# vadimkantorov/convasr

Measured on AMD Instinct MI355X. Metric: audio-seconds/sec/node (fwd+bwd+CTC) at bs64x15s, higher is better.
Workload: dtype bf16

## Files before the change

### convasr_amd/csrc/conv.hip

```cpp
#include "conv_common.h"

template <typename T, bool ALIGNED> __device__ __forceinline__ uint4 load_chunk(const T* row, int e0, int n_valid) {
	constexpr int EPC = 16 / sizeof(T);
	uint4 v = make_uint4(0, 0, 0, 0);
	if (ALIGNED) {
		if (e0 + EPC <= n_valid) v = *reinterpret_cast<const uint4*>(row + e0);
		else if (e0 < n_valid) {
			T tmp[EPC];
#pragma unroll
			for (int i = 0; i < EPC; ++i) tmp[i] = (e0 + i < n_valid) ? row[e0 + i] : (T)0;
			v = *reinterpret_cast<uint4*>(tmp);
		}
	} else if (e0 < n_valid) {
		T tmp[EPC];
#pragma unroll
		for (int i = 0; i < EPC; ++i) tmp[i] = (e0 + i < n_valid) ? row[e0 + i] : (T)0;
		v = *reinterpret_cast<uint4*>(tmp);
	}
	return v;
}

template <typename T, typename O, int XI, bool ALIGNED_X, bool SK = false>
__global__ __launch_bounds__(NTHREADS, sizeof(T) == 4 ? 1 : 2) void conv1d_igemm_kernel(ConvParams p) {
	extern __shared__ __attribute__((aligned(16))) char smem[];
// ... 337 lines not shown
	else return convasr_fail(CONVASR_EUNSUPPORTED, "pack_conv_weight: dtype %d", dtype);
	if (rc) return rc;
	CONVASR_CHECK_LAUNCH("pack_conv_weight");
	return 0;
}

template <typename T, typename O, int XI, bool AL, bool SK = false> static int launch_conv(const ConvParams& p, size_t smem, hipStream_t s) {
	auto kern = conv1d_igemm_kernel<T, O, XI, AL, SK>;
	static unsigned long long attr_set = 0;
	convasr_allow_160k_lds(reinterpret_cast<const void*>(kern), attr_set);
	constexpr int BK = ROW_BYTES / sizeof(T);
	const int splits = SK ? ((p.Cin + BK - 1) / BK + p.cib_per_split - 1) / p.cib_per_split : 1;
	hipLaunchKernelGGL(kern, dim3(p.total_tiles, splits), dim3(NTHREADS), smem, s, p);
	return 0;
}

template <typename T, typename O, bool SK = false> static int dispatch_conv(const ConvParams& p, size_t smem, hipStream_t s) {
	const int xi = (p.x_rows * 8 + NTHREADS - 1) / NTHREADS;
	const bool al = ((p.Cin * sizeof(T)) & 15) == 0;
	if (!al) {
		if (xi <= 9) return launch_conv<T, O, 9, false, SK>(p, smem, s);
		return convasr_fail(CONVASR_EUNSUPPORTED, "conv1d: halo too large (x_rows %d)", p.x_rows);
	}
	if (xi <= 5) return launch_conv<T, O, 5, true, SK>(p, smem, s);
	if (xi <= 9) return launch_conv<T, O, 9, true, SK>(p, smem, s);
	if (xi <= 16) return launch_conv<T, O, 16, true, SK>(p, smem, s);
	return convasr_fail(CONVASR_EUNSUPPORTED, "conv1d: halo too large (x_rows %d)", p.x_rows);
}

int convasr_conv1d_v2_try(ConvParams p, int x_dtype, int y_dtype, hipStream_t s, int* m_tiles_out);
int convasr_conv1x1_try(ConvParams p, int x_dtype, int y_dtype, hipStream_t s, int* rows_out);
int convasr_wgrad_v2_try(WgradParams& p, int dtype, hipStream_t s);
int convasr_wgrad_v2_supports(const WgradParams& p);
static int g_conv_use_v2 = 1;
static int g_conv_debug = 0;
int convasr_conv_debug_bits() { return g_conv_debug; }
extern "C" int convasr_debug_set_conv_v2(int enable) { const int prev = g_conv_use_v2; g_conv_use_v2 = enable & 1; g_conv_debug = enable >> 8; return prev; }

static int conv1d_run(const void* x, const void* wp, void* y, int x_dtype, int y_dtype, int B, int Cin, int Cout, int Tin, int Tout, int K,
                      int stride, int dil, int pad, const float* bias, double* stats, const float* scale, const float* shift, int act,
                      float act_lo, float act_hi, const float* xlen, const ConvParams* bn_fusion, int* rows_out, void* stream) {
	CONVASR_CHECK_ARG(x && wp && y && B > 0 && Cin > 0 && Cout > 0 && Tin > 0 && Tout > 0 && K > 0 && stride > 0 && dil > 0, "conv1d_fwd: bad arguments");
	CONVASR_CHECK_ARG((scale == nullptr) == (shift == nullptr), "conv1d_fwd: scale and shift go together");
	const int64_t expect = ((int64_t)Tin + 2 * (int64_t)pad - (int64_t)dil * (K - 1) - 1) / stride + 1;
	CONVASR_CHECK_ARG(Tout <= expect, "conv1d_fwd: Tout %d inconsistent with Tin %d K %d stride %d dil %d pad %d (at most %lld)", Tout, Tin, K, stride, dil, pad, (long long)expect);
	CONVASR_CHECK_ARG(x_dtype == CONVASR_F32 || convasr_is_half(x_dtype), "conv1d_fwd: x dtype %d", x_dtype);
	if (K == 1 && stride == 1 && pad == 0 && Tin == Tout && B > 1 && !xlen && !(bn_fusion && bn_fusion->bn_xlen) && !(g_conv_debug & 512) &&
	    (int64_t)B * Tin * (Cin > Cout ? Cin : Cout) * 4 < (1ll << 31)) {
		Tin = Tout = B * Tin;
		B = 1;
	}
	ConvParams p = {};
	if (bn_fusion) p = *bn_fusion;
	p.x = x; p.w = wp; p.y = y; p.bias = bias; p.stats = stats; p.scale = scale; p.shift = shift; p.xlen = xlen;
	p.B = B; p.Cin = Cin; p.Cout = Cout; p.CoutPad = convasr_conv_cout_pad(Cout); p.Tin = Tin; p.Tout = Tout; p.K = K; p.stride = stride; p.dil = dil; p.pad = pad;
	p.act = act; p.act_lo = act_lo; p.act_hi = act_hi; p.debug = g_conv_debug;
	p.m_tiles_per_b = (Tout + BM - 1) / BM;
	p.n_tiles = p.CoutPad / BN;
	p.total_tiles = B * p.m_tiles_per_b * p.n_tiles;
	int xr = (BM - 1) * stride + (K - 1) * dil + 1;
	p.x_rows = (xr + 1) & ~1;
	const size_t osz = y_dtype == CONVASR_F32 ? 4 : 2;
	size_t smem = 2 * (size_t)p.x_rows * ROW_BYTES + 2 * BN * ROW_BYTES;
	const size_t epi = (size_t)BM * (BN * osz + 16) + 4 * BN * sizeof(float);
	if (epi > smem) smem = epi;
	CONVASR_CHECK_ARG(smem <= 160 * 1024, "conv1d_fwd: tile needs %zu B of LDS", smem);
// ... 350 lines not shown
	double s = 0;
	for (int i = 0; i < 16; ++i) s += red[i][cl];
	out[c] = accumulate ? out[c] + (float)s : (float)s;
}

extern "C" int64_t convasr_colsum_workspace_bytes(int64_t rows, int C) { return ceil_div64(rows, 256) * (int64_t)C * 4; }
extern "C" int convasr_colsum(const void* y, int dtype, int64_t rows, int C, float* out, void* workspace, int accumulate, void* stream) {
	CONVASR_CHECK_ARG(y && out && workspace && rows > 0 && C > 0 && (dtype == CONVASR_F32 || convasr_is_half(dtype)), "colsum: bad arguments");
	hipStream_t s = (hipStream_t)stream;
	const int rows_per_block = 256;
	dim3 grid((C + 63) / 64, (unsigned)ceil_div64(rows, rows_per_block));
	float* part = (float*)workspace;
	if (dtype == CONVASR_F32) hipLaunchKernelGGL((colsum_kernel<float>), grid, dim3(256), 0, s, (const float*)y, part, rows, C, rows_per_block);
	else if (dtype == CONVASR_F16) hipLaunchKernelGGL((colsum_kernel<f16_t>), grid, dim3(256), 0, s, (const f16_t*)y, part, rows, C, rows_per_block);
	else hipLaunchKernelGGL((colsum_kernel<bf16_t>), grid, dim3(256), 0, s, (const bf16_t*)y, part, rows, C, rows_per_block);
	hipLaunchKernelGGL(colsum_final_kernel, dim3((C + 63) / 64), dim3(1024), 0, s, (const float*)part, (int)grid.y, C, out, accumulate);
	CONVASR_CHECK_LAUNCH("colsum");
	return 0;
}

extern "C" int64_t convasr_conv1d_wgrad_workspace_bytes(int B, int Cin, int Cout, int Tin, int Tout, int K, int stride, int dil) {
	WgradParams p;
	p.debug = 0;
	p.B = B; p.Cin = Cin; p.Cout = Cout; p.Tin = Tin; p.Tout = Tout; p.K = K; p.stride = stride; p.dil = dil;
	p.pad = 0;
	int splits = 1;
	const int bkt[3] = {64, WgTile<bf16_t>::BKT, WgTile<float>::BKT};
	const double us[3] = {1.6, 2.7, 11.0};
	for (int i = 0; i < 3; ++i) {
		WgradParams q = p;
		wgrad_plan(q, bkt[i], us[i]);
		if (q.splits > splits) splits = q.splits;
	}
	const int64_t slabs = (int64_t)splits * K * (int64_t)Cout * Cin * 4;
	const int64_t dbias_parts = ceil_div64((int64_t)B * Tout, 256) * Cout * 4;
	return slabs > dbias_parts ? slabs : dbias_parts;
}

template <typename T, int XI, bool AX, bool AY> static void launch_wgrad(const WgradParams& p, size_t smem, hipStream_t s) {
	auto kern = conv1d_wgrad_kernel<T, XI, AX, AY>;
	static unsigned long long attr_set = 0;
	convasr_allow_160k_lds(reinterpret_cast<const void*>(kern), attr_set);
	hipLaunchKernelGGL(kern, dim3(p.units * p.splits), dim3(NTHREADS), smem, s, p);
}

template <typename T> static int dispatch_wgrad(WgradParams& p, hipStream_t s) {
	wgrad_plan(p, WgTile<T>::BKT, sizeof(T) == 2 ? 2.7 : 11.0);
	const int xi = (p.x_rows * WgTile<T>::CPR + NTHREADS - 1) / NTHREADS;
	const size_t smem = 2 * (size_t)(WgTile<T>::BKT + p.x_rows) * WgTile<T>::PITCH;
	if (smem > 160 * 1024 || xi > 12) return convasr_fail(CONVASR_EUNSUPPORTED, "conv1d_wgrad: tile too large (x_rows %d)", p.x_rows);
	const bool ax = ((p.Cin * sizeof(T)) & 15) == 0, ay = ((p.Cout * sizeof(T)) & 15) == 0;
	if (ax && ay) { if (xi <= 5) launch_wgrad<T, 5, true, true>(p, smem, s); else launch_wgrad<T, 12, true, true>(p, smem, s); }
	else if (ax) launch_wgrad<T, 12, true, false>(p, smem, s);
	else if (ay) launch_wgrad<T, 12, false, true>(p, smem, s);
	else launch_wgrad<T, 12, false, false>(p, smem, s);
	return 0;
}

static int wgrad_impl(const void* x, int x_ld, const void* dy, int dy_ld, float* dw, float* dbias, void* workspace, int dtype, int B, int Cin, int Cout, int Tin,
                      int Tout, int K, int stride, int dil, int pad, int accumulate, int dw_layout, void* stream) {
	CONVASR_CHECK_ARG(x && dy && dw && workspace && B > 0 && Cin > 0 && Cout > 0 && Tin > 0 && Tout > 0 && K > 0 && stride > 0 && dil > 0 && (dw_layout == CONVASR_W_REFERENCE || dw_layout == CONVASR_W_KMAJOR), "conv1d_wgrad: bad arguments");
	CONVASR_CHECK_ARG(dw_layout == CONVASR_W_REFERENCE || (((int64_t)Cout * Cin) & 3) == 0, "conv1d_wgrad: K-major dw needs Cout * Cin %% 4 == 0");
	CONVASR_CHECK_ARG(K <= 64, "conv1d_wgrad: K %d > 64", K);
	WgradParams p;
	p.debug = g_conv_debug;
	p.x = x; p.dy = dy; p.slab = (float*)workspace;
// ... 116 lines not shown
```

### convasr_amd/csrc/conv_common.h

```cpp
#pragma once
#include "common.h"

typedef float f32x16 __attribute__((ext_vector_type(16)));
typedef float f32x4 __attribute__((ext_vector_type(4)));
typedef __bf16 bf16x8 __attribute__((ext_vector_type(8)));
typedef _Float16 f16x8 __attribute__((ext_vector_type(8)));

#define BM 128
#define BN 128
#define NTHREADS 256
#define ROW_BYTES 128

struct ConvParams {
	const void* x;
	const void* w;
	void* y;
	const float* bias;
	double* stats;
	const float* scale;
	const float* shift;
	const float* xlen;
	int B, Cin, Cout, CoutPad, Tin, Tout, K, stride, dil, pad;
	int act;
	float act_lo, act_hi;
// ... 56 lines not shown
};
template <> struct Mma<float> {
	static constexpr int EPC = 4;
	__device__ static __forceinline__ void run(const uint4& a, const uint4& b, f32x16& c) {
		c = __builtin_amdgcn_mfma_f32_32x32x2f32(__uint_as_float(a.x), __uint_as_float(b.x), c, 0, 0, 0);
		c = __builtin_amdgcn_mfma_f32_32x32x2f32(__uint_as_float(a.y), __uint_as_float(b.y), c, 0, 0, 0);
		c = __builtin_amdgcn_mfma_f32_32x32x2f32(__uint_as_float(a.z), __uint_as_float(b.z), c, 0, 0, 0);
		c = __builtin_amdgcn_mfma_f32_32x32x2f32(__uint_as_float(a.w), __uint_as_float(b.w), c, 0, 0, 0);
	}
};


template <typename T> struct Mma16;
template <> struct Mma16<bf16_t> {
	template <typename V> __device__ static __forceinline__ f32x4 run(const V& a, const V& b, const f32x4& c) { return __builtin_amdgcn_mfma_f32_16x16x32_bf16(__builtin_bit_cast(bf16x8, a), __builtin_bit_cast(bf16x8, b), c, 0, 0, 0); }
};
template <> struct Mma16<f16_t> {
	template <typename V> __device__ static __forceinline__ f32x4 run(const V& a, const V& b, const f32x4& c) { return __builtin_amdgcn_mfma_f32_16x16x32_f16(__builtin_bit_cast(f16x8, a), __builtin_bit_cast(f16x8, b), c, 0, 0, 0); }
};


#define WG_TG 4

struct WgradParams {
	const void* x;
	const void* dy;
	float* slab;
	int B, Cin, Cout, Tin, Tout, K, stride, dil, pad;
	int co_tiles, ci_tiles, tap_groups, units, splits;
	int chunks_per_b, total_chunks, chunks_per_split;
	int x_rows;
	int debug;
	int x_ld, dy_ld;
};

typedef short s16x4 __attribute__((ext_vector_type(4)));

#define WGRAD_MAX_SPLITS 32

static inline void wgrad_plan(WgradParams& p, int bkt, double chunk_us) {
	p.co_tiles = (p.Cout + 127) / 128;
	p.ci_tiles = (p.Cin + 127) / 128;
	p.tap_groups = (p.K + WG_TG - 1) / WG_TG;
	p.units = p.co_tiles * p.ci_tiles * p.tap_groups;
	p.chunks_per_b = (p.Tout + bkt - 1) / bkt;
	p.total_chunks = p.B * p.chunks_per_b;
	const double slab_us = 2.0 * p.K * (double)p.Cout * p.Cin * 4.0 / 4e6;
	double best = 1e30;
	int best_s = 1;
	for (int s = 1; s <= WGRAD_MAX_SPLITS && s <= p.total_chunks; ++s) {
		const int cps = (p.total_chunks + s - 1) / s, s_eff = (p.total_chunks + cps - 1) / cps;
		const int rounds = (p.units * s_eff + 255) / 256;
		const double cost = rounds * cps * chunk_us + s_eff * slab_us;
		if (cost < best) { best = cost; best_s = s_eff; }
	}
	p.splits = best_s;
	p.chunks_per_split = (p.total_chunks + best_s - 1) / best_s;
	p.splits = (p.total_chunks + p.chunks_per_split - 1) / p.chunks_per_split;
	const int taps = p.K < WG_TG ? p.K : WG_TG;
	p.x_rows = (bkt - 1) * p.stride + (taps - 1) * p.dil + 1;
}
```

### convasr_amd/csrc/wgrad_v2.hip

```cpp
#include "conv_common.h"
#include <type_traits>

#define W2_THREADS 512
#define W2_ALL_THREADS (512 + 256)
#define W2_BKT 64
#define W2_YBYTES (W2_BKT * 256)

typedef int v4i32 __attribute__((ext_vector_type(4)));

#ifdef CONVASR_STAMPS
__device__ unsigned long long g_w2_stamps[256 * 8 * 8];
extern "C" int convasr_debug_read_wgrad_stamps(unsigned long long* host, int count) {
	return hipMemcpyFromSymbol(host, HIP_SYMBOL(g_w2_stamps), sizeof(unsigned long long) * count) == hipSuccess ? 0 : -1;
}
#define WSTAMP(var) { __builtin_amdgcn_sched_barrier(0); asm volatile("s_memtime %0\n\ts_waitcnt lgkmcnt(0)" : "=s"(var) :: "memory"); __builtin_amdgcn_sched_barrier(0); }
#else
#define WSTAMP(var)
#endif

__device__ __forceinline__ v4i32 w2_make_srd(const char* base, unsigned num_bytes) {
	const unsigned long long a = (unsigned long long)base;
	v4i32 d;
	d[0] = __builtin_amdgcn_readfirstlane((int)(unsigned)a);
	d[1] = __builtin_amdgcn_readfirstlane((int)(unsigned)((a >> 32) & 0xffffu));
	d[2] = __builtin_amdgcn_readfirstlane((int)num_bytes);
	d[3] = 0x00020000;
	return d;
}

__device__ __forceinline__ void w2_dma16(const v4i32& srd, unsigned lds_addr, int voff) {
	unsigned keep;
	asm volatile("s_nop 4\n\ts_mov_b32 %0, m0\n\ts_mov_b32 m0, %3\n\ts_nop 0\n\tbuffer_load_dwordx4 %1, %2, 0 offen lds\n\ts_mov_b32 m0, %0"
	             : "=&s"(keep)
	             : "v"(voff), "s"(srd), "s"(lds_addr)
	             : "memory");
}

__device__ __forceinline__ uint4 w2_tr_frag(const char* p0, const char* p1) {
	typedef __attribute__((address_space(3))) s16x4* lp;
	const s16x4 lo = __builtin_amdgcn_ds_read_tr16_b64_v4i16((lp)p0);
	const s16x4 hi = __builtin_amdgcn_ds_read_tr16_b64_v4i16((lp)p1);
	const uint2 l = __builtin_bit_cast(uint2, lo), h = __builtin_bit_cast(uint2, hi);
	return make_uint4(l.x, l.y, h.x, h.y);
}

#define W2_MAX_GROUP 12
struct WgradGroup {
	WgradParams prob[W2_MAX_GROUP];
	int first[W2_MAX_GROUP + 1];
	int n;
};

template <typename H> __device__ __forceinline__ void wgrad_v2_body(const WgradParams& p, const int v, char* const smem) {
	const int tid = threadIdx.x, lane = tid & 63;
	const int wave = __builtin_amdgcn_readfirstlane(tid >> 6);
	const int tp = wave >> 2, wm = (wave >> 1) & 1, wn = wave & 1;

	const int unit = v % p.units, split = v / p.units;
#ifdef CONVASR_AB_WGRAD_ORDER
	int tg, ci_t, co_t;
	{
		const int order = (p.debug >> 13) & 3;
		if (order == 1) { co_t = unit % p.co_tiles; ci_t = (unit / p.co_tiles) % p.ci_tiles; tg = unit / (p.co_tiles * p.ci_tiles); }
		else if (order == 2) {
			const int BS = 3, cb = (p.co_tiles + BS - 1) / BS, ib = (p.ci_tiles + BS - 1) / BS;
			int u = unit, found = 0; tg = ci_t = co_t = 0;
			for (int b0 = 0; b0 < cb * ib && !found; ++b0) {
				const int c0 = (b0 / ib) * BS, i0 = (b0 % ib) * BS;
				const int nc = min(BS, p.co_tiles - c0), ni = min(BS, p.ci_tiles - i0), n = nc * ni * p.tap_groups;
				if (u < n) { tg = u % p.tap_groups; const int r = u / p.tap_groups; ci_t = i0 + r % ni; co_t = c0 + r / ni; found = 1; }
				else u -= n;
			}
		}
		else { tg = unit % p.tap_groups; ci_t = (unit / p.tap_groups) % p.ci_tiles; co_t = unit / (p.tap_groups * p.ci_tiles); }
	}
#else
	const int tg = unit % p.tap_groups, ci_t = (unit / p.tap_groups) % p.ci_tiles, co_t = unit / (p.tap_groups * p.ci_tiles);
#endif
	const int co0 = co_t * 128, ci0 = ci_t * 128, tap0 = tg * WG_TG;
	const int c_begin = split * p.chunks_per_split, c_end = min(p.total_chunks, c_begin + p.chunks_per_split);
	const int ntaps = min(WG_TG, p.K - tap0);
	int tapA, tapB;
	unsigned mA, mB;
	bool shA = false, shB = false;
	if (ntaps == 4) { tapA = tap0 + 2 * tp; tapB = tapA + 1; mA = 15u; mB = 15u; }
	else if (ntaps == 3) { tapA = tap0 + tp; tapB = tap0 + 2; mA = 15u; mB = tp ? 12u : 3u; shB = true; }
	else if (ntaps == 2) { tapA = tap0 + tp; tapB = tapA; mA = 15u; mB = 0u; }
	else { tapA = tap0; tapB = tap0; mA = tp ? 12u : 3u; mB = 0u; shA = true; }

	const int xbytes = p.x_rows * 256;
	const int stage_bytes = W2_YBYTES + xbytes;
	const unsigned lds_base = (unsigned)(size_t)(__attribute__((address_space(3))) char*)smem;
	const int y_row_bytes = (p.dy_ld ? p.dy_ld : p.Cout) * 2, x_row_bytes = (p.x_ld ? p.x_ld : p.Cin) * 2;
	const int y_pieces = W2_BKT / 4, x_pieces = p.x_rows >> 2, pieces = y_pieces + x_pieces;
	const bool loader = wave >= 8;
	const int lw = wave - 8;
	const int my_pieces = (pieces - lw + 3) >> 2;
	const int prow = lane >> 4, pchunk = (lane & 15) ^ (prow << 2);
	const int ylane = prow * y_row_bytes + pchunk * 16 + co0 * 2, xlane = prow * x_row_bytes + pchunk * 16 + ci0 * 2;

	auto issue = [&](int c, int stage) {
		const int b = c / p.chunks_per_b, t0 = (c % p.chunks_per_b) * W2_BKT;
		const v4i32 ysrd = w2_make_srd(reinterpret_cast<const char*>(p.dy) + (int64_t)b * p.Tout * y_row_bytes, (unsigned)(p.Tout * y_row_bytes));
		const v4i32 xsrd = w2_make_srd(reinterpret_cast<const char*>(p.x) + (int64_t)b * p.Tin * x_row_bytes, (unsigned)(p.Tin * x_row_bytes));
		const unsigned dst = lds_base + stage * stage_bytes;
		const int tin0 = t0 - p.pad + tap0 * p.dil;
		for (int j = lw; j < pieces; j += 4) {
			if (j < y_pieces) w2_dma16(ysrd, __builtin_amdgcn_readfirstlane(dst + j * 1024), (t0 + j * 4) * y_row_bytes + ylane);
			else w2_dma16(xsrd, __builtin_amdgcn_readfirstlane(dst + W2_YBYTES + (j - y_pieces) * 1024), (tin0 + (j - y_pieces) * 4) * x_row_bytes + xlane);
		}
	};

	f32x16 acc[2][2][2];
#pragma unroll
	for (int a = 0; a < 2; ++a)
#pragma unroll
		for (int i = 0; i < 2; ++i)
#pragma unroll
			for (int j = 0; j < 2; ++j)
#pragma unroll
				for (int k = 0; k < 16; ++k) acc[a][i][j][k] = 0.f;

	if (loader) {
		for (int i = 0; i < 3; ++i)
			if (c_begin + i < c_end) issue(c_begin + i, i);
		asm volatile("s_waitcnt vmcnt(0)" ::: "memory");
		__builtin_amdgcn_s_barrier();
		int stage = 0;
		for (int c = c_begin; c < c_end; ++c) {
			const bool more = c + 3 < c_end;
			if (more) issue(c + 3, (stage + 3) & 3);
			if (!more) asm volatile("s_waitcnt vmcnt(0)" ::: "memory");
			else switch (my_pieces) {
				case 10: asm volatile("s_waitcnt vmcnt(10)" ::: "memory"); break;
				case 9: asm volatile("s_waitcnt vmcnt(9)" ::: "memory"); break;
				case 8: asm volatile("s_waitcnt vmcnt(8)" ::: "memory"); break;
				case 7: asm volatile("s_waitcnt vmcnt(7)" ::: "memory"); break;
				case 6: asm volatile("s_waitcnt vmcnt(6)" ::: "memory"); break;
				case 5: asm volatile("s_waitcnt vmcnt(5)" ::: "memory"); break;
				default: asm volatile("s_waitcnt vmcnt(0)" ::: "memory"); break;
			}
			__builtin_amdgcn_s_barrier();
			stage = (stage + 1) & 3;
		}
		if (ntaps == 3 || ntaps == 1) __builtin_amdgcn_s_barrier();
		return;
	}
	__builtin_amdgcn_s_barrier();
#ifdef CONVASR_STAMPS
	unsigned long long wa = 0, wb = 0, wc = 0, w_work = 0, w_bar = 0, w_t0 = 0, w_t1 = 0, w_t2 = 0;
	WSTAMP(w_t0)
#endif

	const int g4 = lane >> 4, q = (lane >> 2) & 3, pc = lane & 3;
	const int krow = 8 * (g4 >> 1) + q;
	const int colA = (wm * 64 + (g4 & 1) * 16 + 4 * pc) * 2, colB = (wn * 64 + (g4 & 1) * 16 + 4 * pc) * 2;
	const int offA = (tapA - tap0) * p.dil, offB = (tapB - tap0) * p.dil;
	auto swz = [](int cb, int r3) { return (((cb >> 6) ^ r3) << 6) | (cb & 63); };
	const unsigned aoff0 = krow * 256 + swz(colA, q), aoff1 = krow * 256 + swz(colA + 64, q);
	const unsigned bAoff0 = W2_YBYTES + (krow + offA) * 256 + swz(colB, (q + offA) & 3), bAoff1 = W2_YBYTES + (krow + offA) * 256 + swz(colB + 64, (q + offA) & 3);
	const unsigned bBoff0 = W2_YBYTES + (krow + offB) * 256 + swz(colB, (q + offB) & 3), bBoff1 = W2_YBYTES + (krow + offB) * 256 + swz(colB + 64, (q + offB) & 3);
	struct F2 { uint4 u0, u1; };
	typedef __attribute__((address_space(3))) s16x4* lp;
	auto tr8 = [](unsigned addr) {
		const s16x4 lo = __builtin_amdgcn_ds_read_tr16_b64_v4i16((lp)(size_t)addr);
		const s16x4 hi = __builtin_amdgcn_ds_read_tr16_b64_v4i16((lp)(size_t)(addr + 4 * 256));
		const uint2 l = __builtin_bit_cast(uint2, lo), h2 = __builtin_bit_cast(uint2, hi);
		return make_uint4(l.x, l.y, h2.x, h2.y);
	};
	auto load_a = [&](unsigned st, int kk, F2& f) { f.u0 = tr8(st + aoff0 + kk * 4096); f.u1 = tr8(st + aoff1 + kk * 4096); };
	auto load_bA = [&](unsigned st, int kk, F2& f) { f.u0 = tr8(st + bAoff0 + kk * 4096); f.u1 = tr8(st + bAoff1 + kk * 4096); };
	auto load_bB = [&](unsigned st, int kk, F2& f) { f.u0 = tr8(st + bBoff0 + kk * 4096); f.u1 = tr8(st + bBoff1 + kk * 4096); };
	auto mma4 = [&](const F2& a, const F2& bq, f32x16 (&c)[2][2]) {
		Mma<H>::run(a.u0, bq.u0, c[0][0]);
		Mma<H>::run(a.u0, bq.u1, c[0][1]);
		Mma<H>::run(a.u1, bq.u0, c[1][0]);
		Mma<H>::run(a.u1, bq.u1, c[1][1]);
	};

	auto chunk_loop = [&](auto MA_, auto MB_) {
		constexpr unsigned MA = decltype(MA_)::value, MB = decltype(MB_)::value, MAB = MA | MB;
		int stage = 0;
		F2 fa0, fa1, fbA, fbB;
		const unsigned st0 = lds_base;
		if (c_begin < c_end) { if (MAB & 1u) load_a(st0, 0, fa0); if (MA & 1u) load_bA(st0, 0, fbA); }
		for (int c = c_begin; c < c_end; ++c) {
			WSTAMP(wa)
			const unsigned st = lds_base + stage * stage_bytes, stn = lds_base + ((stage + 1) & 3) * stage_bytes;
#define W2_DS2_M1 __builtin_amdgcn_sched_group_barrier(0x100, 2, 0); __builtin_amdgcn_sched_group_barrier(0x008, 1, 0);
#define W2_HINT(KK) if (MA == 15u && MB == 15u) { W2_DS2_M1 W2_DS2_M1 __builtin_amdgcn_sched_group_barrier(0x008, 2, 0); W2_DS2_M1 W2_DS2_M1 W2_DS2_M1 W2_DS2_M1 }
#define W2_SUBSTEP(KK, FA_CUR, FA_NXT)                                                                                              \
			if ((MB >> KK) & 1u) load_bB(st, KK, fbB);                                                                                  \
			if ((MA >> KK) & 1u) mma4(FA_CUR, fbA, acc[0]);                                                                             \
			if (KK < 3) { if ((MAB >> ((KK + 1) & 3)) & 1u) load_a(st, KK + 1, FA_NXT); if ((MA >> ((KK + 1) & 3)) & 1u) load_bA(st, KK + 1, fbA); } \
			else { if (MAB & 1u) load_a(stn, 0, FA_NXT); if (MA & 1u) load_bA(stn, 0, fbA); }   \
			if ((MB >> KK) & 1u) mma4(FA_CUR, fbB, acc[1]);                                                                             \
			W2_HINT(KK)
			W2_SUBSTEP(0, fa0, fa1)
			W2_SUBSTEP(1, fa1, fa0)
			W2_SUBSTEP(2, fa0, fa1)
			W2_SUBSTEP(3, fa1, fa0)
#undef W2_SUBSTEP
#undef W2_HINT
#undef W2_DS2_M1
			WSTAMP(wb)
			__builtin_amdgcn_s_barrier();
			WSTAMP(wc)
#ifdef CONVASR_STAMPS
			w_work += wb - wa; w_bar += wc - wb;
#endif
			stage = (stage + 1) & 3;
		}
	};
	typedef std::integral_constant<unsigned, 15u> M15;
	typedef std::integral_constant<unsigned, 12u> M12;
	typedef std::integral_constant<unsigned, 3u> M3;
	typedef std::integral_constant<unsigned, 0u> M0;
	if (ntaps == 4) chunk_loop(M15(), M15());
	else if (ntaps == 3) { if (tp) chunk_loop(M15(), M12()); else chunk_loop(M15(), M3()); }
	else if (ntaps == 2) chunk_loop(M15(), M0());
	else { if (tp) chunk_loop(M12(), M0()); else chunk_loop(M3(), M0()); }

	WSTAMP(w_t1)
	const int r = lane & 31, h = lane >> 5;
	float* const red = reinterpret_cast<float*>(smem) + (wave & 3) * 64 * 64 + lane;
#pragma unroll
	for (int a = 0; a < 2; ++a) {
		const bool shared = a == 0 ? shA : shB;
		const unsigned m = a == 0 ? mA : mB;
		if (shared) {
			if (tp == 1) {
#pragma unroll
				for (int mi = 0; mi < 2; ++mi)
#pragma unroll
					for (int ni = 0; ni < 2; ++ni)
#pragma unroll
						for (int g = 0; g < 16; ++g) red[((mi * 2 + ni) * 16 + g) * 64] = acc[a][mi][ni][g];
			}
			__syncthreads();
			if (tp == 0) {
#pragma unroll
				for (int mi = 0; mi < 2; ++mi)
#pragma unroll
					for (int ni = 0; ni < 2; ++ni)
#pragma unroll
						for (int g = 0; g < 16; ++g) acc[a][mi][ni][g] += red[((mi * 2 + ni) * 16 + g) * 64];
			}
		}
		if (m == 0u || (shared && tp == 1)) continue;
		const int tap = a == 0 ? tapA : tapB;
		float* sl = p.slab + ((int64_t)split * p.K + tap) * p.Cout * p.Cin;
#pragma unroll
		for (int mi = 0; mi < 2; ++mi)
#pragma unroll
			for (int ni = 0; ni < 2; ++ni) {
				const int ci = ci0 + wn * 64 + ni * 32 + r;
#pragma unroll
				for (int g = 0; g < 16; ++g) {
					const int co = co0 + wm * 64 + mi * 32 + (g & 3) + 8 * (g >> 2) + 4 * h;
					sl[(int64_t)co * p.Cin + ci] = acc[a][mi][ni][g];
				}
			}
	}
#ifdef CONVASR_STAMPS
	WSTAMP(w_t2)
	if (blockIdx.x < 256 && lane == 0) {
		unsigned long long* o = g_w2_stamps + (blockIdx.x * 8 + wave) * 8;
		o[0] = w_work; o[1] = w_bar; o[2] = w_t1 - w_t0; o[3] = w_t2 - w_t1; o[4] = (unsigned long long)(c_end - c_begin);
	}
#endif
}

template <typename H> __global__ __launch_bounds__(W2_ALL_THREADS, 3) void conv1d_wgrad_v2_kernel(WgradParams p) {
	extern __shared__ __attribute__((aligned(16))) char smem[];
	wgrad_v2_body<H>(p, xcd_remap(blockIdx.x, p.units * p.splits), smem);
}

template <typename H> __global__ __launch_bounds__(W2_ALL_THREADS, 3) void conv1d_wgrad_v2_grouped_kernel(WgradGroup g) {
	extern __shared__ __attribute__((aligned(16))) char smem[];
	const int v = xcd_remap(blockIdx.x, g.first[g.n]);
	int q = 0;
#pragma unroll
	for (int i = 1; i < W2_MAX_GROUP; ++i) q += (i < g.n && v >= g.first[i]) ? 1 : 0;
	q = __builtin_amdgcn_readfirstlane(q);
	wgrad_v2_body<H>(g.prob[q], v - g.first[q], smem);
}

static size_t wgrad_v2_plan(const WgradParams& p, WgradParams& q) {
	if (p.stride != 1 || (p.Cin & 127) != 0 || (p.Cout & 127) != 0) return 0;
	if ((int64_t)p.Tin * (p.x_ld ? p.x_ld : p.Cin) * 2 >= (1ll << 31) || (int64_t)p.Tout * (p.dy_ld ? p.dy_ld : p.Cout) * 2 >= (1ll << 31)) return 0;
	if ((p.x_ld & 7) || (p.dy_ld & 7)) return 0;
	q = p;
	wgrad_plan(q, W2_BKT, 1.6);
	q.x_rows = (q.x_rows + 3) & ~3;
	const int pieces = W2_BKT / 4 + q.x_rows / 4;
	if (pieces > 40) return 0;
	const size_t smem = 4 * (size_t)(W2_YBYTES + q.x_rows * 256);
	return smem > 160 * 1024 ? 0 : smem;
}

int convasr_wgrad_v2_supports(const WgradParams& p) {
	WgradParams q;
	return wgrad_v2_plan(p, q) != 0;
}

int convasr_wgrad_v2_try(WgradParams& p, int dtype, hipStream_t s) {
	WgradParams q;
	const size_t smem = wgrad_v2_plan(p, q);
	if (!smem) return 0;
	const bool f16 = dtype == CONVASR_F16;
	const void* kern = f16 ? (const void*)conv1d_wgrad_v2_kernel<f16_t> : (const void*)conv1d_wgrad_v2_kernel<bf16_t>;
	static unsigned long long set[2] = {0, 0};
	convasr_allow_160k_lds(kern, set[f16]);
	void* args[] = {&q};
	if (hipLaunchKernel(kern, dim3(q.units * q.splits), dim3(W2_ALL_THREADS), args, smem, s) != hipSuccess) { (void)hipGetLastError(); return 0; }
	p = q;
	return 1;
}

struct WgradCombine {
	const float* slab[W2_MAX_GROUP]; float* dw[W2_MAX_GROUP]; float* zero[W2_MAX_GROUP];
	long long first4[W2_MAX_GROUP + 1];
	int zero_n[W2_MAX_GROUP];
	int accumulate[W2_MAX_GROUP];
	int n, S;
};

__global__ __launch_bounds__(256) void wgrad_reduce_grouped_kernel(WgradCombine c) {
	const long long total = c.first4[c.n];
	for (long long i = (long long)blockIdx.x * 256 + threadIdx.x; i < total; i += (long long)gridDim.x * 256) {
		int q = 0;
#pragma unroll
		for (int k = 1; k < W2_MAX_GROUP; ++k) q += (k < c.n && i >= c.first4[k]) ? 1 : 0;
		const long long j = i - c.first4[q], n4 = c.first4[q + 1] - c.first4[q];
		const float4* const s4 = reinterpret_cast<const float4*>(c.slab[q]);
		float4 a = s4[j];
		for (int s = 1; s < c.S; ++s) { const float4 b = s4[(long long)s * n4 + j]; a.x += b.x; a.y += b.y; a.z += b.z; a.w += b.w; }
		float4* const d4 = reinterpret_cast<float4*>(c.dw[q]);
		if (c.accumulate[q]) { const float4 o = d4[j]; a.x += o.x; a.y += o.y; a.z += o.z; a.w += o.w; }
		d4[j] = a;
	}
	if (blockIdx.x == 0)
		for (int q = 0; q < c.n; ++q)
			if (c.zero[q])
				for (int k = threadIdx.x; k < c.zero_n[q]; k += 256) c.zero[q][k] = 0.f;
}

static void wgrad_group_plan(WgradParams* probs, int n) {
	for (int i = 0; i < n; ++i) {
		WgradParams& p = probs[i];
		p.co_tiles = p.Cout / 128; p.ci_tiles = p.Cin / 128; p.tap_groups = 1; p.units = p.co_tiles * p.ci_tiles;
		p.chunks_per_b = (p.Tout + W2_BKT - 1) / W2_BKT; p.total_chunks = p.B * p.chunks_per_b;
		p.x_rows = W2_BKT;
	}
	const int total_chunks = probs[0].total_chunks;
	int units = 0; double slab_us = 0;
	for (int i = 0; i < n; ++i) { units += probs[i].units; slab_us += 2.0 * (double)probs[i].Cout * probs[i].Cin * 4.0 / 4e6; }
	double best = 1e30; int best_s = 1;
	for (int s = 1; s <= WGRAD_MAX_SPLITS && s <= total_chunks; ++s) {
		const int cps = (total_chunks + s - 1) / s, s_eff = (total_chunks + cps - 1) / cps;
		const int rounds = (units * s_eff + 255) / 256;
		const double cost = rounds * cps * 1.6 + s_eff * slab_us;
		if (cost < best) { best = cost; best_s = s_eff; }
	}
	for (int i = 0; i < n; ++i) {
		WgradParams& p = probs[i];
		p.chunks_per_split = (total_chunks + best_s - 1) / best_s;
		p.splits = (total_chunks + p.chunks_per_split - 1) / p.chunks_per_split;
	}
}

extern "C" int64_t convasr_wgrad1x1_grouped_workspace_bytes(int n, const int* cin, const int* cout, int B, int T) {
	if (n <= 0 || n > W2_MAX_GROUP || !cin || !cout || B <= 0 || T <= 0) return -1;
	WgradParams probs[W2_MAX_GROUP];
	for (int i = 0; i < n; ++i) { probs[i] = WgradParams(); probs[i].B = B; probs[i].Cin = cin[i]; probs[i].Cout = cout[i]; probs[i].Tin = probs[i].Tout = T; probs[i].K = 1; probs[i].stride = probs[i].dil = 1; }
	wgrad_group_plan(probs, n);
	int64_t bytes = 0;
	for (int i = 0; i < n; ++i) bytes += (int64_t)probs[i].splits * cout[i] * cin[i] * 4;
	return bytes;
}

extern "C" int convasr_wgrad1x1_grouped(int n, const void* const* x, const void* const* dy, float* const* dw, float* const* zero, const int* cin, const int* cout,
                                        const int* accumulate, void* workspace, int dtype, int B, int T, void* stream) {
	CONVASR_CHECK_ARG(n > 0 && n <= W2_MAX_GROUP && x && dy && dw && cin && cout && workspace && B > 0 && T > 0, "wgrad1x1_grouped: bad arguments (at most %d problems)", W2_MAX_GROUP);
	if (!convasr_is_half(dtype)) return convasr_fail(CONVASR_EUNSUPPORTED, "wgrad1x1_grouped: dtype %d (16-bit storage only)", dtype);
	WgradGroup g = {};
	WgradCombine c = {};
	for (int i = 0; i < n; ++i) {
		CONVASR_CHECK_ARG(x[i] && dy[i] && dw[i], "wgrad1x1_grouped: problem %d has a NULL operand", i);
		if ((cin[i] & 127) || (cout[i] & 127) || cin[i] <= 0 || cout[i] <= 0 || (int64_t)T * cin[i] * 2 >= (1ll << 31) || (int64_t)T * cout[i] * 2 >= (1ll << 31))
			return convasr_fail(CONVASR_EUNSUPPORTED, "wgrad1x1_grouped: problem %d (%d x %d channels) is outside the kernel's envelope (channel counts %% 128)", i, cout[i], cin[i]);
		WgradParams& p = g.prob[i];
		p = WgradParams();
		p.x = x[i]; p.dy = dy[i]; p.B = B; p.Cin = cin[i]; p.Cout = cout[i]; p.Tin = p.Tout = T; p.K = 1; p.stride = p.dil = 1; p.pad = 0; p.debug = 0;
	}
	wgrad_group_plan(g.prob, n);
	g.n = c.n = n;
	c.S = g.prob[0].splits;
	float* slab = (float*)workspace;
	for (int i = 0; i < n; ++i) {
		g.prob[i].slab = slab;
		c.slab[i] = slab; c.dw[i] = dw[i]; c.zero[i] = zero ? zero[i] : nullptr; c.zero_n[i] = cout[i]; c.accumulate[i] = accumulate ? accumulate[i] : 0;
		c.first4[i + 1] = c.first4[i] + (long long)cout[i] * cin[i] / 4;
		slab += (int64_t)g.prob[i].splits * cout[i] * cin[i];
		g.first[i + 1] = g.first[i] + g.prob[i].units * g.prob[i].splits;
	}
	const size_t smem = 4 * (size_t)(W2_YBYTES + W2_BKT * 256);
	const bool f16 = dtype == CONVASR_F16;
	const void* kern = f16 ? (const void*)conv1d_wgrad_v2_grouped_kernel<f16_t> : (const void*)conv1d_wgrad_v2_grouped_kernel<bf16_t>;
	static unsigned long long set[2] = {0, 0};
	convasr_allow_160k_lds(kern, set[f16]);
	hipStream_t s = (hipStream_t)stream;
	void* args[] = {&g};
	if (hipLaunchKernel(kern, dim3(g.first[n]), dim3(W2_ALL_THREADS), args, smem, s) != hipSuccess) return convasr_fail(CONVASR_ELAUNCH, "wgrad1x1_grouped: %s", hipGetErrorString(hipGetLastError()));
	long long blocks = (c.first4[n] + 255) / 256;
	if (blocks > 2048) blocks = 2048;
	hipLaunchKernelGGL(wgrad_reduce_grouped_kernel, dim3((unsigned)blocks), dim3(256), 0, s, c);
	CONVASR_CHECK_LAUNCH("wgrad1x1_grouped");
	return 0;
}
```

Baseline: 59580.

## Add wide 1x1 wgrad mode covering two Cin tiles per block with a 3-stage ring

For K=1 weight-gradient problems, each block now computes two adjacent 128-wide Cin tiles, and the two tap-pair wave groups each take one tile. This replaces the half-idle single-tap masking, so each loaded dy chunk is reused across twice the Cin width. To fit in LDS, the wide path uses a 3-stage ring and loads the next stage's first fragment after the barrier instead of prefetching it. The split planner now uses the real CU count and a different per-chunk cost, and workspace sizing takes the maximum over modes. The risks are fewer blocks (lower parallelism), a shallower pipeline, and more LDS per block.

Measured after the change: 59860 (median of 6 runs). About the same (+0.5%).

```diff
diff --git a/convasr_amd/csrc/conv.hip b/convasr_amd/csrc/conv.hip
--- a/convasr_amd/csrc/conv.hip
+++ b/convasr_amd/csrc/conv.hip
@@ -393,6 +393,7 @@
 int convasr_conv1x1_try(ConvParams p, int x_dtype, int y_dtype, hipStream_t s, int* rows_out);
 int convasr_wgrad_v2_try(WgradParams& p, int dtype, hipStream_t s);
 int convasr_wgrad_v2_supports(const WgradParams& p);
+int convasr_wgrad_v2_max_splits(WgradParams p);
 static int g_conv_use_v2 = 1;
 static int g_conv_debug = 0;
 int convasr_conv_debug_bits() { return g_conv_debug; }
@@ -809,6 +810,9 @@
 		wgrad_plan(q, bkt[i], us[i]);
 		if (q.splits > splits) splits = q.splits;
 	}
+	p.x_ld = p.dy_ld = 0;
+	const int v2 = convasr_wgrad_v2_max_splits(p);
+	if (v2 > splits) splits = v2;
 	const int64_t slabs = (int64_t)splits * K * (int64_t)Cout * Cin * 4;
 	const int64_t dbias_parts = ceil_div64((int64_t)B * Tout, 256) * Cout * 4;
 	return slabs > dbias_parts ? slabs : dbias_parts;
diff --git a/convasr_amd/csrc/conv_common.h b/convasr_amd/csrc/conv_common.h
--- a/convasr_amd/csrc/conv_common.h
+++ b/convasr_amd/csrc/conv_common.h
@@ -112,6 +112,7 @@
 	int x_rows;
 	int debug;
 	int x_ld, dy_ld;
+	int ci_units, wide;
 };
 
 typedef short s16x4 __attribute__((ext_vector_type(4)));
diff --git a/convasr_amd/csrc/wgrad_v2.hip b/convasr_amd/csrc/wgrad_v2.hip
--- a/convasr_amd/csrc/wgrad_v2.hip
+++ b/convasr_amd/csrc/wgrad_v2.hip
@@ -51,7 +51,7 @@
 	int n;
 };
 
-template <typename H> __device__ __forceinline__ void wgrad_v2_body(const WgradParams& p, const int v, char* const smem) {
+template <typename H, bool WIDE> __device__ __forceinline__ void wgrad_v2_unit(const WgradParams& p, const int v, char* const smem) {
 	const int tid = threadIdx.x, lane = tid & 63;
 	const int wave = __builtin_amdgcn_readfirstlane(tid >> 6);
 	const int tp = wave >> 2, wm = (wave >> 1) & 1, wn = wave & 1;
@@ -74,8 +74,11 @@
 		}
 		else { tg = unit % p.tap_groups; ci_t = (unit / p.tap_groups) % p.ci_tiles; co_t = unit / (p.tap_groups * p.ci_tiles); }
 	}
+	constexpr bool wide = false;
 #else
-	const int tg = unit % p.tap_groups, ci_t = (unit / p.tap_groups) % p.ci_tiles, co_t = unit / (p.tap_groups * p.ci_tiles);
+	const int cj = (unit / p.tap_groups) % p.ci_units;
+	const int tg = unit % p.tap_groups, ci_t = p.wide ? 2 * cj : cj, co_t = unit / (p.tap_groups * p.ci_units);
+	constexpr bool wide = WIDE;
 #endif
 	const int co0 = co_t * 128, ci0 = ci_t * 128, tap0 = tg * WG_TG;
 	const int c_begin = split * p.chunks_per_split, c_end = min(p.total_chunks, c_begin + p.chunks_per_split);
@@ -86,13 +89,14 @@
 	if (ntaps == 4) { tapA = tap0 + 2 * tp; tapB = tapA + 1; mA = 15u; mB = 15u; }
 	else if (ntaps == 3) { tapA = tap0 + tp; tapB = tap0 + 2; mA = 15u; mB = tp ? 12u : 3u; shB = true; }
 	else if (ntaps == 2) { tapA = tap0 + tp; tapB = tapA; mA = 15u; mB = 0u; }
+	else if (wide) { tapA = tap0; tapB = tap0; mA = 15u; mB = 0u; }
 	else { tapA = tap0; tapB = tap0; mA = tp ? 12u : 3u; mB = 0u; shA = true; }
 
 	const int xbytes = p.x_rows * 256;
-	const int stage_bytes = W2_YBYTES + xbytes;
+	const int stage_bytes = W2_YBYTES + (wide ? 2 * xbytes : xbytes);
 	const unsigned lds_base = (unsigned)(size_t)(__attribute__((address_space(3))) char*)smem;
 	const int y_row_bytes = (p.dy_ld ? p.dy_ld : p.Cout) * 2, x_row_bytes = (p.x_ld ? p.x_ld : p.Cin) * 2;
-	const int y_pieces = W2_BKT / 4, x_pieces = p.x_rows >> 2, pieces = y_pieces + x_pieces;
+	const int y_pieces = W2_BKT / 4, x_pieces = p.x_rows >> 2, pieces = y_pieces + (wide ? 2 * x_pieces : x_pieces);
 	const bool loader = wave >= 8;
 	const int lw = wave - 8;
 	const int my_pieces = (pieces - lw + 3) >> 2;
@@ -107,7 +111,10 @@
 		const int tin0 = t0 - p.pad + tap0 * p.dil;
 		for (int j = lw; j < pieces; j += 4) {
 			if (j < y_pieces) w2_dma16(ysrd, __builtin_amdgcn_readfirstlane(dst + j * 1024), (t0 + j * 4) * y_row_bytes + ylane);
-			else w2_dma16(xsrd, __builtin_amdgcn_readfirstlane(dst + W2_YBYTES + (j - y_pieces) * 1024), (tin0 + (j - y_pieces) * 4) * x_row_bytes + xlane);
+			else {
+				const int xj = j - y_pieces, second = wide && xj >= x_pieces ? 1 : 0, r = xj - second * x_pieces;
+				w2_dma16(xsrd, __builtin_amdgcn_readfirstlane(dst + W2_YBYTES + xj * 1024), (tin0 + r * 4) * x_row_bytes + second * 256 + xlane);
+			}
 		}
 	};
 
@@ -122,16 +129,19 @@
 				for (int k = 0; k < 16; ++k) acc[a][i][j][k] = 0.f;
 
 	if (loader) {
-		for (int i = 0; i < 3; ++i)
+		constexpr int ring = wide ? 3 : 4, ahead = ring - 1;
+		for (int i = 0; i < ahead; ++i)
 			if (c_begin + i < c_end) issue(c_begin + i, i);
 		asm volatile("s_waitcnt vmcnt(0)" ::: "memory");
 		__builtin_amdgcn_s_barrier();
 		int stage = 0;
 		for (int c = c_begin; c < c_end; ++c) {
-			const bool more = c + 3 < c_end;
-			if (more) issue(c + 3, (stage + 3) & 3);
+			const bool more = c + ahead < c_end;
+			if (more) issue(c + ahead, ring == 4 ? ((stage + ahead) & 3) : (stage + ahead >= ring ? stage + ahead - ring : stage + ahead));
 			if (!more) asm volatile("s_waitcnt vmcnt(0)" ::: "memory");
 			else switch (my_pieces) {
+				case 12: asm volatile("s_waitcnt vmcnt(12)" ::: "memory"); break;
+				case 11: asm volatile("s_waitcnt vmcnt(11)" ::: "memory"); break;
 				case 10: asm volatile("s_waitcnt vmcnt(10)" ::: "memory"); break;
 				case 9: asm volatile("s_waitcnt vmcnt(9)" ::: "memory"); break;
 				case 8: asm volatile("s_waitcnt vmcnt(8)" ::: "memory"); break;
@@ -141,9 +151,9 @@
 				default: asm volatile("s_waitcnt vmcnt(0)" ::: "memory"); break;
 			}
 			__builtin_amdgcn_s_barrier();
-			stage = (stage + 1) & 3;
+			stage = ring == 4 ? ((stage + 1) & 3) : (stage + 1 == ring ? 0 : stage + 1);
 		}
-		if (ntaps == 3 || ntaps == 1) __builtin_amdgcn_s_barrier();
+		if (shA || shB) __builtin_amdgcn_s_barrier();
 		return;
 	}
 	__builtin_amdgcn_s_barrier();
@@ -158,7 +168,8 @@
 	const int offA = (tapA - tap0) * p.dil, offB = (tapB - tap0) * p.dil;
 	auto swz = [](int cb, int r3) { return (((cb >> 6) ^ r3) << 6) | (cb & 63); };
 	const unsigned aoff0 = krow * 256 + swz(colA, q), aoff1 = krow * 256 + swz(colA + 64, q);
-	const unsigned bAoff0 = W2_YBYTES + (krow + offA) * 256 + swz(colB, (q + offA) & 3), bAoff1 = W2_YBYTES + (krow + offA) * 256 + swz(colB + 64, (q + offA) & 3);
+	const unsigned xtile = wide ? W2_YBYTES + tp * xbytes : W2_YBYTES;
+	const unsigned bAoff0 = xtile + (krow + offA) * 256 + swz(colB, (q + offA) & 3), bAoff1 = xtile + (krow + offA) * 256 + swz(colB + 64, (q + offA) & 3);
 	const unsigned bBoff0 = W2_YBYTES + (krow + offB) * 256 + swz(colB, (q + offB) & 3), bBoff1 = W2_YBYTES + (krow + offB) * 256 + swz(colB + 64, (q + offB) & 3);
 	struct F2 { uint4 u0, u1; };
 	typedef __attribute__((address_space(3))) s16x4* lp;
@@ -178,22 +189,24 @@
 		Mma<H>::run(a.u1, bq.u1, c[1][1]);
 	};
 
-	auto chunk_loop = [&](auto MA_, auto MB_) {
+	auto chunk_loop = [&](auto MA_, auto MB_, auto RING_) {
 		constexpr unsigned MA = decltype(MA_)::value, MB = decltype(MB_)::value, MAB = MA | MB;
+		constexpr int RING = decltype(RING_)::value;
+		constexpr bool PRE = RING == 4;
 		int stage = 0;
 		F2 fa0, fa1, fbA, fbB;
 		const unsigned st0 = lds_base;
 		if (c_begin < c_end) { if (MAB & 1u) load_a(st0, 0, fa0); if (MA & 1u) load_bA(st0, 0, fbA); }
 		for (int c = c_begin; c < c_end; ++c) {
 			WSTAMP(wa)
-			const unsigned st = lds_base + stage * stage_bytes, stn = lds_base + ((stage + 1) & 3) * stage_bytes;
+			const unsigned st = lds_base + stage * stage_bytes, stn = lds_base + (RING == 4 ? ((stage + 1) & 3) : (stage + 1 == RING ? 0 : stage + 1)) * stage_bytes;
 #define W2_DS2_M1 __builtin_amdgcn_sched_group_barrier(0x100, 2, 0); __builtin_amdgcn_sched_group_barrier(0x008, 1, 0);
 #define W2_HINT(KK) if (MA == 15u && MB == 15u) { W2_DS2_M1 W2_DS2_M1 __builtin_amdgcn_sched_group_barrier(0x008, 2, 0); W2_DS2_M1 W2_DS2_M1 W2_DS2_M1 W2_DS2_M1 }
 #define W2_SUBSTEP(KK, FA_CUR, FA_NXT)                                                                                              \
 			if ((MB >> KK) & 1u) load_bB(st, KK, fbB);                                                                                  \
 			if ((MA >> KK) & 1u) mma4(FA_CUR, fbA, acc[0]);                                                                             \
 			if (KK < 3) { if ((MAB >> ((KK + 1) & 3)) & 1u) load_a(st, KK + 1, FA_NXT); if ((MA >> ((KK + 1) & 3)) & 1u) load_bA(st, KK + 1, fbA); } \
-			else { if (MAB & 1u) load_a(stn, 0, FA_NXT); if (MA & 1u) load_bA(stn, 0, fbA); }   \
+			else if (PRE) { if (MAB & 1u) load_a(stn, 0, FA_NXT); if (MA & 1u) load_bA(stn, 0, fbA); }   \
 			if ((MB >> KK) & 1u) mma4(FA_CUR, fbB, acc[1]);                                                                             \
 			W2_HINT(KK)
 			W2_SUBSTEP(0, fa0, fa1)
@@ -205,21 +218,25 @@
 #undef W2_DS2_M1
 			WSTAMP(wb)
 			__builtin_amdgcn_s_barrier();
+			if (!PRE) { if (MAB & 1u) load_a(stn, 0, fa0); if (MA & 1u) load_bA(stn, 0, fbA); }
 			WSTAMP(wc)
 #ifdef CONVASR_STAMPS
 			w_work += wb - wa; w_bar += wc - wb;
 #endif
-			stage = (stage + 1) & 3;
+			stage = RING == 4 ? ((stage + 1) & 3) : (stage + 1 == RING ? 0 : stage + 1);
 		}
 	};
 	typedef std::integral_constant<unsigned, 15u> M15;
 	typedef std::integral_constant<unsigned, 12u> M12;
 	typedef std::integral_constant<unsigned, 3u> M3;
 	typedef std::integral_constant<unsigned, 0u> M0;
-	if (ntaps == 4) chunk_loop(M15(), M15());
-	else if (ntaps == 3) { if (tp) chunk_loop(M15(), M12()); else chunk_loop(M15(), M3()); }
-	else if (ntaps == 2) chunk_loop(M15(), M0());
-	else { if (tp) chunk_loop(M12(), M0()); else chunk_loop(M3(), M0()); }
+	typedef std::integral_constant<int, 4> R4;
+	typedef std::integral_constant<int, 3> R3;
+	if (wide) chunk_loop(M15(), M0(), R3());
+	else if (ntaps == 4) chunk_loop(M15(), M15(), R4());
+	else if (ntaps == 3) { if (tp) chunk_loop(M15(), M12(), R4()); else chunk_loop(M15(), M3(), R4()); }
+	else if (ntaps == 2) chunk_loop(M15(), M0(), R4());
+	else { if (tp) chunk_loop(M12(), M0(), R4()); else chunk_loop(M3(), M0(), R4()); }
 
 	WSTAMP(w_t1)
 	const int r = lane & 31, h = lane >> 5;
@@ -254,7 +271,7 @@
 		for (int mi = 0; mi < 2; ++mi)
 #pragma unroll
 			for (int ni = 0; ni < 2; ++ni) {
-				const int ci = ci0 + wn * 64 + ni * 32 + r;
+				const int ci = ci0 + (wide ? tp * 128 : 0) + wn * 64 + ni * 32 + r;
 #pragma unroll
 				for (int g = 0; g < 16; ++g) {
 					const int co = co0 + wm * 64 + mi * 32 + (g & 3) + 8 * (g >> 2) + 4 * h;
@@ -271,6 +288,13 @@
 #endif
 }
 
+template <typename H> __device__ __forceinline__ void wgrad_v2_body(const WgradParams& p, const int v, char* const smem) {
+#ifndef CONVASR_AB_WGRAD_ORDER
+	if (p.wide && 2 * (((v % p.units) / p.tap_groups) % p.ci_units) + 1 < p.ci_tiles) { wgrad_v2_unit<H, true>(p, v, smem); return; }
+#endif
+	wgrad_v2_unit<H, false>(p, v, smem);
+}
+
 template <typename H> __global__ __launch_bounds__(W2_ALL_THREADS, 3) void conv1d_wgrad_v2_kernel(WgradParams p) {
 	extern __shared__ __attribute__((aligned(16))) char smem[];
 	wgrad_v2_body<H>(p, xcd_remap(blockIdx.x, p.units * p.splits), smem);
@@ -284,6 +308,42 @@
 	for (int i = 1; i < W2_MAX_GROUP; ++i) q += (i < g.n && v >= g.first[i]) ? 1 : 0;
 	q = __builtin_amdgcn_readfirstlane(q);
 	wgrad_v2_body<H>(g.prob[q], v - g.first[q], smem);
+}
+
+static int w2_pick_splits(int total_chunks, int units, double chunk_us, double slab_us, int* cps_out) {
+	const int n_cu = convasr_cu_count();
+	double best = 1e30; int best_s = 1;
+	for (int s = 1; s <= WGRAD_MAX_SPLITS && s <= total_chunks; ++s) {
+		const int cps = (total_chunks + s - 1) / s, s_eff = (total_chunks + cps - 1) / cps;
+		const int rounds = (units * s_eff + n_cu - 1) / n_cu;
+		const double cost = rounds * cps * chunk_us + s_eff * slab_us;
+		if (cost < best) { best = cost; best_s = s_eff; }
+	}
+	const int cps = (total_chunks + best_s - 1) / best_s;
+	*cps_out = cps;
+	return (total_chunks + cps - 1) / cps;
+}
+
+#define W2_WIDE_CHUNK_US 1.1
+
+int convasr_conv_debug_bits();
+static bool w2_regroup_one_tap(WgradParams& q, int debug) {
+	q.wide = 0;
+	q.ci_units = q.ci_tiles;
+#ifndef CONVASR_AB_WGRAD_ORDER
+	const int wide_units = q.co_tiles * ((q.ci_tiles + 1) / 2), max_splits = q.total_chunks < WGRAD_MAX_SPLITS ? q.total_chunks : WGRAD_MAX_SPLITS;
+	if (q.K == 1 && q.ci_tiles >= 2 && !(debug & 262144) && ((debug & 524288) || (int64_t)wide_units * max_splits >= convasr_cu_count())) {
+		q.wide = 1;
+		q.ci_units = (q.ci_tiles + 1) / 2;
+	}
+#endif
+	q.units = q.co_tiles * q.ci_units * q.tap_groups;
+	return q.wide != 0;
+}
+
+static size_t w2_lds_bytes(const WgradParams& q) {
+	const size_t narrow = 4 * (size_t)(W2_YBYTES + q.x_rows * 256), wide = 3 * (size_t)(W2_YBYTES + 2 * q.x_rows * 256);
+	return q.wide && wide > narrow ? wide : narrow;
 }
 
 static size_t wgrad_v2_plan(const WgradParams& p, WgradParams& q) {
@@ -295,13 +355,24 @@
 	q.x_rows = (q.x_rows + 3) & ~3;
 	const int pieces = W2_BKT / 4 + q.x_rows / 4;
 	if (pieces > 40) return 0;
-	const size_t smem = 4 * (size_t)(W2_YBYTES + q.x_rows * 256);
+	if (w2_regroup_one_tap(q, p.debug)) q.splits = w2_pick_splits(q.total_chunks, q.units, W2_WIDE_CHUNK_US, 2.0 * (double)q.Cout * q.Cin * 4.0 / 4e6, &q.chunks_per_split);
+	const size_t smem = w2_lds_bytes(q);
 	return smem > 160 * 1024 ? 0 : smem;
 }
 
 int convasr_wgrad_v2_supports(const WgradParams& p) {
 	WgradParams q;
 	return wgrad_v2_plan(p, q) != 0;
+}
+
+int convasr_wgrad_v2_max_splits(WgradParams p) {
+	int splits = 0;
+	for (int mode = 0; mode < 3; ++mode) {
+		WgradParams q;
+		p.debug = mode * 262144;
+		if (wgrad_v2_plan(p, q) && q.splits > splits) splits = q.splits;
+	}
+	return splits;
 }
 
 int convasr_wgrad_v2_try(WgradParams& p, int dtype, hipStream_t s) {
@@ -346,38 +417,34 @@
 				for (int k = threadIdx.x; k < c.zero_n[q]; k += 256) c.zero[q][k] = 0.f;
 }
 
-static void wgrad_group_plan(WgradParams* probs, int n) {
+static void wgrad_group_plan(WgradParams* probs, int n, int debug) {
+	bool wide = false;
 	for (int i = 0; i < n; ++i) {
 		WgradParams& p = probs[i];
-		p.co_tiles = p.Cout / 128; p.ci_tiles = p.Cin / 128; p.tap_groups = 1; p.units = p.co_tiles * p.ci_tiles;
+		p.co_tiles = p.Cout / 128; p.ci_tiles = p.Cin / 128; p.tap_groups = 1;
 		p.chunks_per_b = (p.Tout + W2_BKT - 1) / W2_BKT; p.total_chunks = p.B * p.chunks_per_b;
 		p.x_rows = W2_BKT;
-	}
-	const int total_chunks = probs[0].total_chunks;
+		if (w2_regroup_one_tap(p, debug)) wide = true;
+	}
 	int units = 0; double slab_us = 0;
 	for (int i = 0; i < n; ++i) { units += probs[i].units; slab_us += 2.0 * (double)probs[i].Cout * probs[i].Cin * 4.0 / 4e6; }
-	double best = 1e30; int best_s = 1;
-	for (int s = 1; s <= WGRAD_MAX_SPLITS && s <= total_chunks; ++s) {
-		const int cps = (total_chunks + s - 1) / s, s_eff = (total_chunks + cps - 1) / cps;
-		const int rounds = (units * s_eff + 255) / 256;
-		const double cost = rounds * cps * 1.6 + s_eff * slab_us;
-		if (cost < best) { best = cost; best_s = s_eff; }
-	}
-	for (int i = 0; i < n; ++i) {
-		WgradParams& p = probs[i];
-		p.chunks_per_split = (total_chunks + best_s - 1) / best_s;
-		p.splits = (total_chunks + p.chunks_per_split - 1) / p.chunks_per_split;
-	}
+	int cps = 1;
+	const int splits = w2_pick_splits(probs[0].total_chunks, units, wide ? W2_WIDE_CHUNK_US : 1.6, slab_us, &cps);
+	for (int i = 0; i < n; ++i) { probs[i].chunks_per_split = cps; probs[i].splits = splits; }
 }
 
 extern "C" int64_t convasr_wgrad1x1_grouped_workspace_bytes(int n, const int* cin, const int* cout, int B, int T) {
 	if (n <= 0 || n > W2_MAX_GROUP || !cin || !cout || B <= 0 || T <= 0) return -1;
-	WgradParams probs[W2_MAX_GROUP];
-	for (int i = 0; i < n; ++i) { probs[i] = WgradParams(); probs[i].B = B; probs[i].Cin = cin[i]; probs[i].Cout = cout[i]; probs[i].Tin = probs[i].Tout = T; probs[i].K = 1; probs[i].stride = probs[i].dil = 1; }
-	wgrad_group_plan(probs, n);
-	int64_t bytes = 0;
-	for (int i = 0; i < n; ++i) bytes += (int64_t)probs[i].splits * cout[i] * cin[i] * 4;
-	return bytes;
+	int64_t most = 0;
+	for (int mode = 0; mode < 3; ++mode) {
+		WgradParams probs[W2_MAX_GROUP];
+		for (int i = 0; i < n; ++i) { probs[i] = WgradParams(); probs[i].B = B; probs[i].Cin = cin[i]; probs[i].Cout = cout[i]; probs[i].Tin = probs[i].Tout = T; probs[i].K = 1; probs[i].stride = probs[i].dil = 1; }
+		wgrad_group_plan(probs, n, mode * 262144);
+		int64_t bytes = 0;
+		for (int i = 0; i < n; ++i) bytes += (int64_t)probs[i].splits * cout[i] * cin[i] * 4;
+		if (bytes > most) most = bytes;
+	}
+	return most;
 }
 
 extern "C" int convasr_wgrad1x1_grouped(int n, const void* const* x, const void* const* dy, float* const* dw, float* const* zero, const int* cin, const int* cout,
@@ -394,7 +461,7 @@
 		p = WgradParams();
 		p.x = x[i]; p.dy = dy[i]; p.B = B; p.Cin = cin[i]; p.Cout = cout[i]; p.Tin = p.Tout = T; p.K = 1; p.stride = p.dil = 1; p.pad = 0; p.debug = 0;
 	}
-	wgrad_group_plan(g.prob, n);
+	wgrad_group_plan(g.prob, n, convasr_conv_debug_bits());
 	g.n = c.n = n;
 	c.S = g.prob[0].splits;
 	float* slab = (float*)workspace;
@@ -405,7 +472,8 @@
 		slab += (int64_t)g.prob[i].splits * cout[i] * cin[i];
 		g.first[i + 1] = g.first[i] + g.prob[i].units * g.prob[i].splits;
 	}
-	const size_t smem = 4 * (size_t)(W2_YBYTES + W2_BKT * 256);
+	size_t smem = 0;
+	for (int i = 0; i < n; ++i) { const size_t b = w2_lds_bytes(g.prob[i]); if (b > smem) smem = b; }
 	const bool f16 = dtype == CONVASR_F16;
 	const void* kern = f16 ? (const void*)conv1d_wgrad_v2_grouped_kernel<f16_t> : (const void*)conv1d_wgrad_v2_grouped_kernel<bf16_t>;
 	static unsigned long long set[2] = {0, 0};
```
